# wearable-motion-capture/arm-pose-estimation

Measured on AMD Instinct MI355X. Metric: IMU windows/sec, higher is better.
Workload: dtype f32; 1 GPU; BASELINE configs[2]: watch_phone_pocket_lstm path, 1024 windows/GPU x 64 frames x 22 features (I=22,H=256,L=2,O=14), z-score+LSTM+head+denorm+FK, inputs resident in HBM; windows_per_gpu=1024, frames=64, features=22

## Files before the change

arm-pose-estimation_amd/csrc/lstm_cluster32.hip:

```cpp
#include <type_traits>

#include "ape_internal.h"
#include "async_look.h"
#include "../../include/ape_hip.h"

namespace {

typedef float f32x16 __attribute__((ext_vector_type(16)));
typedef unsigned u32x4 __attribute__((__vector_size__(4 * sizeof(unsigned))));
constexpr unsigned SPIN_LIMIT = 1u << 22;

#ifdef APE_CLUSTER_STAMPS
#define C32_TL(i) do { if (p.dbg_wg != nullptr && tid == 0 && cluster == 0 && member == 0 && (i) < 200) p.dbg_wg[256 + (i)] = __builtin_readcyclecounter(); } while (0)
#else
#define C32_TL(i) do {} while (0)
#endif

__device__ __forceinline__ float sigm(float v) { return __builtin_amdgcn_rcpf(1.0f + __builtin_amdgcn_exp2f(-1.4426950408889634f * v)); }
__device__ __forceinline__ float tanh_(float v) { return 2.0f * __builtin_amdgcn_rcpf(1.0f + __builtin_amdgcn_exp2f(-2.885390081777927f * v)) - 1.0f; }

template <bool AG>
__device__ __forceinline__ void mfma32(f32x16& acc, float w, float a) {
    if constexpr (AG) asm volatile("v_mfma_f32_32x32x2_f32 %0, %1, %2, %0" : "+v"(acc) : "a"(w), "v"(a));
    else asm volatile("v_mfma_f32_32x32x2_f32 %0, %1, %2, %0" : "+v"(acc) : "v"(w), "v"(a));
}
__device__ __forceinline__ void mfma_drain(f32x16& acc) { asm volatile("s_nop 15\n\ts_nop 7" : "+v"(acc)); }
template <bool AG>
__device__ __forceinline__ void mfma16(f32x16& acc, const u32x4& w, const u32x4& b) {
    if constexpr (AG) asm volatile("v_mfma_f32_32x32x16_f16 %0, %1, %2, %0" : "+v"(acc) : "a"(w), "v"(b));
    else asm volatile("v_mfma_f32_32x32x16_f16 %0, %1, %2, %0" : "+v"(acc) : "v"(w), "v"(b));
}

template <int NB, bool AG, int NW, typename Mid>
__device__ __forceinline__ void span32(f32x16& acc, const float* __restrict__ src, int stride, const float (&w)[NW], int w0, Mid&& mid) {
    f32x4 a0 = *reinterpret_cast<const f32x4*>(src);
    f32x4 a1 = (NB > 1) ? *reinterpret_cast<const f32x4*>(src + stride) : a0;
    f32x4 a2 = a1;
#pragma unroll
    for (int kb = 0; kb < NB; ++kb) {
        if (kb + 2 < NB) a2 = *reinterpret_cast<const f32x4*>(src + stride * (kb + 2));
#pragma unroll
        for (int j = 0; j < 4; ++j) mfma32<AG>(acc, w[w0 + 4 * kb + j], a0[j]);
        mid(kb);
        a0 = a1;
        a1 = a2;
    }
}

template <int NS, bool AG, int NG, typename Mid>
__device__ __forceinline__ void span16(f32x16& acc, const float* __restrict__ src, const u32x4 (&w)[NG], int g0, Mid&& mid) {
    constexpr int SL = 2 * 2 * 32 * 4;
    u32x4 h0 = *reinterpret_cast<const u32x4*>(src), l0 = *reinterpret_cast<const u32x4*>(src + 128);
    u32x4 h1 = (NS > 1) ? *reinterpret_cast<const u32x4*>(src + SL) : h0, l1 = (NS > 1) ? *reinterpret_cast<const u32x4*>(src + SL + 128) : l0;
    u32x4 h2 = h1, l2 = l1;
#pragma unroll
    for (int s = 0; s < NS; ++s) {
        if (s + 2 < NS) {
            h2 = *reinterpret_cast<const u32x4*>(src + SL * (s + 2));
            l2 = *reinterpret_cast<const u32x4*>(src + SL * (s + 2) + 128);
        }
        mfma16<AG>(acc, w[g0 + 2 * s], h0);
        mfma16<AG>(acc, w[g0 + 2 * s], l0);
        mid(2 * s);
        mfma16<AG>(acc, w[g0 + 2 * s + 1], h0);
        mid(2 * s + 1);
        h0 = h1; l0 = l1;
        h1 = h2; l1 = l2;
    }
}

template <bool HOT>
__device__ __forceinline__ void dma_1k(unsigned lds_addr, unsigned voff, u32x4 rsrc, unsigned soff, int piece_bytes) {
    if constexpr (HOT) {
        unsigned tmp;
        asm volatile("s_add_i32 m0, %1, %5\n\ts_add_i32 %0, %4, %5\n\tbuffer_load_dwordx4 %2, %3, %0 offen sc1 lds"
                     : "=&s"(tmp) : "s"(lds_addr), "v"(voff), "s"(rsrc), "s"(soff), "i"(piece_bytes) : "memory");
    } else {
        asm volatile("s_mov_b32 m0, %0\n\ts_nop 3\n\tbuffer_load_dwordx4 %1, %2, %3 offen sc1 lds"
                     :: "s"(lds_addr + (unsigned)piece_bytes), "v"(voff), "s"(rsrc), "s"(soff + (unsigned)piece_bytes) : "memory");
    }
}


#ifndef C32_QF
#define C32_QF 3
#endif
#ifndef C32_QPD
#define C32_QPD 0
#endif
template <int H, int L, int KX, bool ENDS, int BXU>
__global__ __launch_bounds__(256, 1) void ape_lstm_cluster32(const ClusterParams p) {
    constexpr int UPW = 8;
    constexpr int GH = H / (4 * UPW);
    constexpr int MR = 32;
    constexpr int SX = KX + 4;
    constexpr int BX = KX / 8, BH = H / 8;
    constexpr int NW0 = 4 * (BX + BH);
    constexpr int NW1 = 4 * (2 * BH);
    constexpr int NFL = 4 * GH;
    constexpr int HL = GH * 4 * MR * 8;
    constexpr int NDMA = HL * 4 / 1024 / 4;
    static_assert(H == 256 && L == 2 && KX == 32 && GH == 8 && NDMA == 8, "built for the 2 x 256 models");
    static_assert(BXU == BX || (BXU == BX - 1 && !ENDS), "the short-window instantiation keeps the four-block input span");

    const int tid = threadIdx.x;
    const int lane = tid & 63;
    const int wave = __builtin_amdgcn_readfirstlane(tid >> 6);
    const int n = lane & 31, hh = lane >> 5;
    const int T = p.T, I = p.I, O = p.O;
    const bool normalize = (p.flags & APE_FLAG_NORMALIZE_INPUT) != 0;
    const bool bcast_x = (p.flags & APE_FLAG_BROADCAST_X) != 0;

    extern __shared__ __attribute__((aligned(16))) float smem[];
    float* hb0 = smem;
    float* hb1 = hb0 + 2 * HL;
    float* xin = hb1 + HL;
    f32x4* bias_s = reinterpret_cast<f32x4*>(xin + MR * SX);
    unsigned* look_s = reinterpret_cast<unsigned*>(bias_s + 4 * L * 4 * 64);
    int* ctl = reinterpret_cast<int*>(look_s + 4 * 64);

    unsigned* const class_ticket = p.xcc_slots + 64;
    unsigned* const xcc_words = p.xcc_slots + 64 + 8 * 16;
    const int cls = blockIdx.x & 7;
    unsigned my_xcc;
    asm volatile("s_getreg_b32 %0, hwreg(HW_REG_XCC_ID)" : "=s"(my_xcc));
    my_xcc &= 0xFu;
    if (tid == 0) {
        ctl[0] = 0;
        ctl[1] = -1;
        if (__hip_atomic_load(p.status, __ATOMIC_RELAXED, __HIP_MEMORY_SCOPE_AGENT) == 0u) {
            const unsigned tk = __hip_atomic_fetch_add(class_ticket + cls * 16, 1u, __ATOMIC_RELAXED, __HIP_MEMORY_SCOPE_AGENT);
            if (tk < gridDim.x / 8) ctl[1] = (int)tk;
            else __hip_atomic_store(p.status, 2u, __ATOMIC_RELAXED, __HIP_MEMORY_SCOPE_AGENT);
        }
    }
    __syncthreads();
    if (ctl[1] < 0) return;
    const int ticket = __builtin_amdgcn_readfirstlane(ctl[1]);
    const int cluster = (ticket / GH) * 8 + cls, member = ticket % GH;
    const int row0 = cluster * MR;
    C32_TL(0);
    if (tid == 0)
        __hip_atomic_store(xcc_words + cluster * GH + member, 0x10u | my_xcc, __ATOMIC_RELAXED, __HIP_MEMORY_SCOPE_AGENT);

    constexpr int NE = (MR * KX) / 256;
    const int xk = tid % KX, xrow = tid / KX;
    const int rows_here = bcast_x ? MR : max(0, min(MR, p.B - row0));
    const unsigned long long x_addr = reinterpret_cast<unsigned long long>(p.x + (bcast_x ? (size_t)0 : (size_t)row0 * T * I));
    const unsigned x_lo = __builtin_amdgcn_readfirstlane((unsigned)x_addr), x_hi = __builtin_amdgcn_readfirstlane((unsigned)(x_addr >> 32));
    const int x_bytes = __builtin_amdgcn_readfirstlane((int)((size_t)(bcast_x ? 1 : rows_here) * T * I * sizeof(float)));
    const __amdgpu_buffer_rsrc_t x_rsrc = __builtin_amdgcn_make_buffer_rsrc(
        reinterpret_cast<float*>(((unsigned long long)x_hi << 32) | x_lo), 0, x_bytes, 0x00020000);
    const unsigned x_rowbytes = bcast_x ? 0u : (unsigned)(T * I * sizeof(float));
    const unsigned x_off0 = (xk < I) ? (unsigned)xrow * x_rowbytes + (unsigned)(xk * sizeof(float)) : 0x80000000u;
    const unsigned x_estride = (unsigned)(256 / KX) * x_rowbytes;
    float xr[NE];
    auto fetch_x = [&](int t) {
        const int slot = (t + p.x_ring >= T) ? t + p.x_ring - T : t + p.x_ring;
#pragma unroll
        for (int e = 0; e < NE; ++e) {
            const unsigned off = (xrow + e * (256 / KX) < rows_here) ? x_off0 + (unsigned)e * x_estride : 0x80000000u;
            xr[e] = __builtin_bit_cast(float, __builtin_amdgcn_raw_buffer_load_b32(x_rsrc, off, (unsigned)(slot * I * sizeof(float)), 0));
        }
    };
    double x_mean = (normalize && xk < I) ? p.xx_m[xk] : 0.0;
    double x_std = (normalize && xk < I) ? p.xx_s[xk] : 1.0;
    double x_rstd = (normalize && xk < I) ? p.xx_r[xk] : 1.0;
    asm volatile("" : "+v"(x_mean), "+v"(x_std), "+v"(x_rstd));
    auto stage_x = [&]() {
#pragma unroll
        for (int e = 0; e < NE; ++e) {
            const double d = (double)xr[e] - x_mean;
            const double q0 = d * x_rstd;
            const double rr = fma(-q0, x_std, d);
            const double q1 = fma(rr, x_rstd, q0);
            xin[(xrow + e * (256 / KX)) * SX + xk] = (float)((rr == rr) ? q1 : q0);
        }
    };
    fetch_x(0);

    float w0[4 * BXU];
    u32x4 w0h[NW0 / 4 - BX];
    u32x4 w1[NW1 / 4];
    const f32x4* const s0 = reinterpret_cast<const f32x4*>(p.wcl[0]) + ((size_t)(member * 4 + wave) * (NW0 / 4)) * 64 + lane;
    const u32x4* const s1 = reinterpret_cast<const u32x4*>(p.wcl[1]) + ((size_t)(member * 4 + wave) * (NW1 / 4)) * 64 + lane;
#pragma unroll
    for (int i = 0; i < BXU; ++i) {
        const f32x4 v = s0[i * 64];
        w0[4 * i] = v[0]; w0[4 * i + 1] = v[1]; w0[4 * i + 2] = v[2]; w0[4 * i + 3] = v[3];
    }
    auto load_weights = [&]() {
#pragma unroll
        for (int i = BX; i < NW0 / 4; ++i) w0h[i - BX] = reinterpret_cast<const u32x4*>(s0)[i * 64];
#pragma unroll
        for (int i = 0; i < NW1 / 4; ++i) w1[i] = s1[i * 64];
    };
#pragma unroll
    for (int l = 0; l < L; ++l)
#pragma unroll
        for (int gate = 0; gate < 4; ++gate) {
            f32x4 bv;
#pragma unroll
            for (int j = 0; j < 4; ++j) bv[j] = p.bias[l][gate * H + member * 32 + wave * 8 + 4 * hh + j] * p.gate_scale[l];
            bias_s[((wave * L + l) * 4 + gate) * 64 + lane] = bv;
        }
    float cst[L][4];
#pragma unroll
    for (int l = 0; l < L; ++l)
#pragma unroll
        for (int j = 0; j < 4; ++j) cst[l][j] = 0.0f;

    const __amdgpu_buffer_rsrc_t hx_rsrc = __builtin_amdgcn_make_buffer_rsrc(p.hx, 0, (int)p.hx_bytes, 0x00020000);
    const unsigned long long hx_addr = reinterpret_cast<unsigned long long>(p.hx);
    u32x4 hx_desc;
    hx_desc[0] = __builtin_amdgcn_readfirstlane((unsigned)hx_addr);
    hx_desc[1] = __builtin_amdgcn_readfirstlane((unsigned)(hx_addr >> 32) & 0xFFFFu);
    hx_desc[2] = __builtin_amdgcn_readfirstlane((unsigned)p.hx_bytes);
    hx_desc[3] = 0x00020000u;
    unsigned* const flags_of = p.xflags + (size_t)cluster * L * NFL;
    const ape_desc_t fl_desc = ape_make_desc(p.xflags, (unsigned)((gridDim.x / GH) * L * NFL * sizeof(unsigned)));
    const unsigned fl_off = (unsigned)(cluster * L * NFL * sizeof(unsigned));
    const unsigned look_voff = (unsigned)((lane & (NFL - 1)) * sizeof(unsigned));
    const unsigned look_lds = (unsigned)reinterpret_cast<unsigned long long>(look_s) + (unsigned)(wave * 256);
    const unsigned* const look_mine = look_s + wave * 64 + lane;
    constexpr unsigned SET_BYTES = HL * sizeof(float);
    auto hx_base = [&](int l, int par) -> unsigned { return (unsigned)((((size_t)cluster * L + l) * 2 + par) * SET_BYTES); };
    const unsigned hb0_lds = (unsigned)reinterpret_cast<unsigned long long>(hb0);
    const unsigned hb1_lds = (unsigned)reinterpret_cast<unsigned long long>(hb1);

    stage_x();
    if (T > 1) fetch_x(1);

    if (wave == 0) {
        unsigned spins = 0, v = 0u;
        while (true) {
            v = 0x10u | my_xcc;
            if (lane < GH) v = __hip_atomic_load(xcc_words + cluster * GH + lane, __ATOMIC_RELAXED, __HIP_MEMORY_SCOPE_AGENT);
            if (__all((int)(v != 0u))) break;
            if (++spins > SPIN_LIMIT || __hip_atomic_load(p.status, __ATOMIC_RELAXED, __HIP_MEMORY_SCOPE_AGENT) != 0u) {
                if (lane == 0) {
                    ctl[0] = 1;
                    __hip_atomic_store(p.status, 1u, __ATOMIC_RELAXED, __HIP_MEMORY_SCOPE_AGENT);
                }
                break;
            }
            __builtin_amdgcn_s_sleep(2);
        }
        const int same = __all((int)((v & 0xFu) == my_xcc));
        if (lane == 0) ctl[3] = same;
    }
    __syncthreads();
    if (ctl[0] != 0) return;
    C32_TL(1);
    const bool in_l2 = APE_HANDOVER_IN_L2(p.flags, ctl[3] != 0);

    auto wait_flags = [&](int l, unsigned want) {
        unsigned spins = 0;
        while (true) {
            unsigned v = want;
            if (lane < NFL) v = __hip_atomic_load(flags_of + l * NFL + lane, __ATOMIC_RELAXED, __HIP_MEMORY_SCOPE_AGENT);
            if (__all((int)(v >= want))) return;
            if (++spins > SPIN_LIMIT || __hip_atomic_load(p.status, __ATOMIC_RELAXED, __HIP_MEMORY_SCOPE_AGENT) != 0u) {
                if (lane == 0) {
                    ctl[0] = 1;
                    __hip_atomic_store(p.status, 1u, __ATOMIC_RELAXED, __HIP_MEMORY_SCOPE_AGENT);
                }
                return;
            }
            __builtin_amdgcn_s_sleep(1);
        }
    };
    const unsigned dma_voff = (unsigned)(lane * 16);
    auto opaque = [](unsigned v) -> unsigned { asm volatile("" : "+s"(v)); return v; };
    const unsigned wave_kib = (unsigned)(wave * 1024);
    auto issue_piece = [&](auto hot_tag, int l, int step, int k) {
        constexpr bool HOT = decltype(hot_tag)::value;
        const unsigned wk = HOT ? wave_kib : opaque(wave_kib);
        const unsigned src = hx_base(l, step & 1) + wk;
        const unsigned dst = (l == 0 ? hb0_lds + (unsigned)((step & 1) * SET_BYTES) : hb1_lds) + wk;
        dma_1k<HOT>(dst, dma_voff, hx_desc, src, k * 4096);
    };
    constexpr std::true_type HOT{};
    constexpr std::false_type COLD{};
    int pend_idx = -1;
    unsigned pend_epoch = 0u;
    auto raise_pending = [&]() {
        if (pend_idx < 0) return;
        if (lane == 0) __hip_atomic_store(flags_of + pend_idx, pend_epoch, __ATOMIC_RELAXED, __HIP_MEMORY_SCOPE_AGENT);
        pend_idx = -1;
    };
    auto bar = [&]() { asm volatile("s_waitcnt lgkmcnt(0)\n\ts_barrier" ::: "memory"); };

    auto cell_update = [&](const f32x16& acc, int l, float (&c_)[4], float (&hn)[4]) {
        const float ks = -1.4426950408889634f * p.gate_descale[l], kt = -2.885390081777927f * p.gate_descale[l];
#pragma unroll
        for (int j = 0; j < 4; j += 2) {
            typedef float f32x2 __attribute__((ext_vector_type(2)));
            auto exp2_2 = [](f32x2 v) { return f32x2{__builtin_amdgcn_exp2f(v[0]), __builtin_amdgcn_exp2f(v[1])}; };
            auto rcp_2 = [](f32x2 v) { return f32x2{__builtin_amdgcn_rcpf(v[0]), __builtin_amdgcn_rcpf(v[1])}; };
            const f32x2 ai = {acc[j], acc[j + 1]}, af = {acc[4 + j], acc[5 + j]}, ag = {acc[8 + j], acc[9 + j]}, ao = {acc[12 + j], acc[13 + j]};
            const f32x2 iv = rcp_2(1.0f + exp2_2(ks * ai));
            const f32x2 fv = rcp_2(1.0f + exp2_2(ks * af));
            const f32x2 gv = 2.0f * rcp_2(1.0f + exp2_2(kt * ag)) - 1.0f;
            const f32x2 ov = rcp_2(1.0f + exp2_2(ks * ao));
            const f32x2 c = fv * f32x2{c_[j], c_[j + 1]} + iv * gv;
            c_[j] = c[0]; c_[j + 1] = c[1];
            const f32x2 h = ov * (2.0f * rcp_2(1.0f + exp2_2(-2.885390081777927f * c)) - 1.0f);
            hn[j] = h[0]; hn[j + 1] = h[1];
        }
    };
    const unsigned pub_off = (unsigned)((((member * 4 + wave) * MR + n) * 8 + 4 * hh) * sizeof(float));
    const unsigned pub_off_split = (unsigned)(((member * 4 + wave) * 2 * MR + hh * MR + n) * 16);
    auto split_h = [&](const float (&h)[4]) -> u32x4 {
        unsigned hw[2], lw[2];
#pragma unroll
        for (int d = 0; d < 2; ++d) {
            const float a = h[2 * d] * (float)(1 << APE_C32_HSHIFT), b = h[2 * d + 1] * (float)(1 << APE_C32_HSHIFT);
            const _Float16 ah = (_Float16)a, bh = (_Float16)b;
            const _Float16 al = (_Float16)(a - (float)ah), bl = (_Float16)(b - (float)bh);
            hw[d] = (unsigned)__builtin_bit_cast(unsigned short, ah) | ((unsigned)__builtin_bit_cast(unsigned short, bh) << 16);
            lw[d] = (unsigned)__builtin_bit_cast(unsigned short, al) | ((unsigned)__builtin_bit_cast(unsigned short, bl) << 16);
        }
        u32x4 r;
#pragma unroll
        for (int d = 0; d < 2; ++d) {
            const auto sw = __builtin_amdgcn_permlane32_swap(hw[d], lw[d], false, false);
            r[d] = sw[0];
            r[2 + d] = sw[1];
        }
        return r;
    };

    if constexpr (!ENDS) {
        load_weights();
    } else {
        f32x16 acc;
#pragma unroll
        for (int gate = 0; gate < 4; ++gate) {
            const f32x4 bv = bias_s[((wave * L + 0) * 4 + gate) * 64 + lane];
            acc[4 * gate] = bv[0]; acc[4 * gate + 1] = bv[1]; acc[4 * gate + 2] = bv[2]; acc[4 * gate + 3] = bv[3];
        }
        span32<BXU, false, 4 * BXU>(acc, xin + n * SX + hh * 4, 8, w0, 0, [&](int) {});
        mfma_drain(acc);
        float h0[4];
        cell_update(acc, 0, cst[0], h0);
        const u32x4 hv = split_h(h0);
        if (in_l2) __builtin_amdgcn_raw_buffer_store_b128(hv, hx_rsrc, hx_base(0, 0) + pub_off_split, 0, 0);
        else __builtin_amdgcn_raw_buffer_store_b128(hv, hx_rsrc, hx_base(0, 0) + pub_off_split, 0, 16 );
        asm volatile("s_waitcnt vmcnt(0)" ::: "memory");
        if (lane == 0) __hip_atomic_store(flags_of + member * 4 + wave, 1u, __ATOMIC_RELAXED, __HIP_MEMORY_SCOPE_AGENT);
        asm volatile("" ::: "memory");
        load_weights();
        bar();
        if (1 < T) {
            stage_x();
            if (2 < T) fetch_x(2);
        }
    }
    C32_TL(2);

    const int P = T + L - 1;
    bool prefetched = false;
#ifdef APE_C32_COUNTS
    unsigned lc_block[2] = {0u, 0u}, lc_go[2] = {0u, 0u}, lc_n[2] = {0u, 0u};
    unsigned long long lc_top[2] = {0ull, 0ull}, lc_t0 = 0ull;
    const unsigned long long lc_start = __builtin_amdgcn_s_memtime();
#endif
#ifdef APE_CLUSTER_STAMPS
    unsigned long long dg_block[2] = {0, 0}, dg_go[2] = {0, 0};
    unsigned long long dgh[2][6] = {};
    unsigned long long dgc[2][5] = {};
    auto now = [&]() -> unsigned long long {
        const unsigned long long c = __builtin_readcyclecounter();
        asm volatile("s_waitcnt lgkmcnt(0)" ::: "memory");
        return c;
    };
#endif
    auto section = [&](auto steady_tag, auto layer_tag, auto mode_tag, const int ph) -> bool {
        constexpr bool ST = decltype(steady_tag)::value;
        constexpr int l = decltype(layer_tag)::value;
        constexpr int MODE = decltype(mode_tag)::value;
        static_assert(MODE == 0 || (l == L - 1 && (MODE == 3 || !ST)), "the special forms are layer 1's");
        const int t = ph - l;
        const bool active = ST || (t >= 0 && t < T);
        const bool need = ST || (t >= 1 && t <= T);
#ifdef APE_CLUSTER_STAMPS
        const unsigned long long c0 = ST ? now() : 0ull;
#endif
#ifdef APE_C32_COUNTS
        lc_t0 = __builtin_amdgcn_s_memtime();
#endif
        if (MODE == 3) {
        } else if (need) {
            if (!prefetched) {
#ifdef APE_CLUSTER_STAMPS
                dg_block[l] += 1;
#endif
#ifdef APE_C32_COUNTS
                lc_block[l] += 1u;
#endif
                asm volatile("s_waitcnt vmcnt(0)" ::: "memory");
                raise_pending();
                wait_flags(l, (unsigned)t);
#pragma unroll
                for (int k = 0; k < NDMA; ++k) issue_piece(COLD, l, t - 1, k);
                asm volatile("s_waitcnt vmcnt(0)" ::: "memory");
            } else {
                asm volatile("s_waitcnt vmcnt(1)" ::: "memory");
            }
        }
        prefetched = false;
#ifdef APE_CLUSTER_STAMPS
        const unsigned long long c1 = ST ? now() : 0ull;
#endif
        if constexpr (MODE != 3) bar();
#ifdef APE_CLUSTER_STAMPS
        const unsigned long long c2 = ST ? now() : 0ull;
#endif
#ifdef APE_C32_COUNTS
        if (ST && MODE != 3) { lc_top[l] += __builtin_amdgcn_s_memtime() - lc_t0; lc_n[l] += 1u; }
#endif
        const int abort_word = (MODE == 3) ? 0 : ctl[0];
        C32_TL(8 + 2 * (2 * ph + l));
        constexpr int ln = (l + 1 < L) ? l + 1 : 0;
        const int tn = (l + 1 < L) ? t - 1 : t + L;
        const bool pre = (l == L - 1) && (ST || (tn >= 1 && tn <= T));
        unsigned peek = (unsigned)tn;
        bool go = false;
        constexpr int NBL = (l == 0) ? BXU + BH : 2 * BH;
        constexpr int QF = C32_QF, QP = (MODE == 1) ? 16 : NBL / 2 - 2 + C32_QPD, QJ = (MODE == 1) ? 20 : NBL / 2 + 2 + C32_QPD;
        bool staged = false;
#ifdef APE_CLUSTER_STAMPS
        unsigned long long hk0 = 0, hk_free = 0;
#define HK_BEGIN() do { if (ST) hk0 = now(); } while (0)
#define HK_END(k) do { if (ST) dgh[l][k] += now() - hk0; } while (0)
#else
#define HK_BEGIN() do {} while (0)
#define HK_END(k) do {} while (0)
#endif
        auto mid = [&](int q) {
#ifdef APE_CLUSTER_STAMPS
            if (ST && q == QF + 2) hk_free = now();
            if (ST && q == QF + 10) dgh[l][5] += now() - hk_free;
#endif
            if (q == QF) {
                HK_BEGIN();
                asm volatile("s_waitcnt vmcnt(0)" ::: "memory");
                raise_pending();
                HK_END(0);
            }
            if (l == L - 1 && q == ((MODE == 3) ? BH + 1 : QF + 1) && (ST || ph + 1 < T)) {
                HK_BEGIN();
                stage_x();
                if (ST || ph + 2 < T) fetch_x(ph + 2);
                staged = true;
                HK_END(1);
            }
            if constexpr (l == L - 1) {
                if (q == QP) look_issue(look_lds, look_voff, fl_desc, fl_off + (unsigned)(ln * NFL * sizeof(unsigned)));
                if (q == QJ - 1) {
                    look_landed();
                    peek = *look_mine;
                }
                if (q == QJ) {
                    HK_BEGIN();
                    go = pre && __all((int)(peek >= (unsigned)tn)) != 0;
                    HK_END(2);
                }
                if (q >= QJ && q < QJ + NDMA && go) {
                    HK_BEGIN();
                    issue_piece(HOT, ln, tn - 1, q - QJ);
                    HK_END(3);
                }
            }
        };
        float hnew[4] = {0.0f, 0.0f, 0.0f, 0.0f};
        if (active) {
            f32x16 acc;
#pragma unroll
            for (int gate = 0; gate < 4; ++gate) {
                const f32x4 bv = bias_s[((wave * L + l) * 4 + gate) * 64 + lane];
                acc[4 * gate] = bv[0]; acc[4 * gate + 1] = bv[1]; acc[4 * gate + 2] = bv[2]; acc[4 * gate + 3] = bv[3];
            }
            const int frag = hh * 2 * MR * 4 + n * 4;
            if constexpr (l == 0) {
                span32<BXU, false, 4 * BXU>(acc, xin + n * SX + hh * 4, 8, w0, 0, [&](int q) { mid(q); });
                if (ST || t > 0) span16<BH / 2, false, NW0 / 4 - BX>(acc, hb0 + ((t - 1) & 1) * HL + frag, w0h, 0, [&](int q) { mid(BXU + q); });
            } else if constexpr (MODE == 3) {
                constexpr int QO = QF + 1, QO2 = QO + 12;
                static_assert(QO2 + 4 + NDMA <= QP && QP < BH, "the own gather's hooks sit in front of the look for the next section");
                unsigned pk = (unsigned)t;
                bool got1 = false, got2 = false;
                span16<BH / 2, true, NW1 / 4>(acc, hb0 + (t & 1) * HL + frag, w1, 0, [&](int q) {
                    mid(q);
                    if (q == QO) look_issue(look_lds, look_voff, fl_desc, fl_off + (unsigned)(l * NFL * sizeof(unsigned)));
                    if (q == QO + 3) {
                        look_landed();
                        pk = *look_mine;
                    }
                    if (q == QO + 4) got1 = __all((int)(pk >= (unsigned)t)) != 0;
                    if (q >= QO + 4 && q < QO + 4 + NDMA && got1) issue_piece(HOT, l, t - 1, q - (QO + 4));
                    if constexpr (!ST) {
                        if (q == QO2 && !got1) look_issue(look_lds, look_voff, fl_desc, fl_off + (unsigned)(l * NFL * sizeof(unsigned)));
                        if (q == QO2 + 3 && !got1) {
                            look_landed();
                            pk = *look_mine;
                        }
                        if (q == QO2 + 4 && !got1) got2 = __all((int)(pk >= (unsigned)t)) != 0;
                        if (q >= QO2 + 4 && q < QO2 + 4 + NDMA && got2) issue_piece(HOT, l, t - 1, q - (QO2 + 4));
                    }
                });
#ifdef APE_C32_COUNTS
                lc_t0 = __builtin_amdgcn_s_memtime();
#endif
                if (!got1 && !got2) {
#ifdef APE_CLUSTER_STAMPS
                    dg_block[l] += 1;
#endif
#ifdef APE_C32_COUNTS
                    lc_block[l] += 1u;
#endif
                    asm volatile("s_waitcnt vmcnt(0)" ::: "memory");
                    raise_pending();
                    wait_flags(l, (unsigned)t);
#pragma unroll
                    for (int k = 0; k < NDMA; ++k) issue_piece(COLD, l, t - 1, k);
                }
                asm volatile("s_waitcnt vmcnt(0)" ::: "memory");
                bar();
#ifdef APE_C32_COUNTS
                if (ST) { lc_top[l] += __builtin_amdgcn_s_memtime() - lc_t0; lc_n[l] += 1u; }
#endif
                if (ctl[0] != 0) return false;
                span16<BH / 2, true, NW1 / 4>(acc, hb1 + frag, w1, BH, [&](int q) { mid(BH + q); });
            } else {
                span16<BH / 2, true, NW1 / 4>(acc, hb0 + (t & 1) * HL + frag, w1, 0, [&](int q) { mid(q); });
                if (ST || t > 0) span16<BH / 2, true, NW1 / 4>(acc, hb1 + frag, w1, BH, [&](int q) { mid(BH + q); });
            }
#ifdef APE_CLUSTER_STAMPS
            const unsigned long long c3 = ST ? now() : 0ull;
            if (ST) { dgc[l][0] += c1 - c0; dgc[l][1] += c2 - c1; dgc[l][2] += c3 - c2; }
#endif
            mfma_drain(acc);
            cell_update(acc, l, cst[l], hnew);
        }
        if (abort_word != 0) return false;
        if (!ST && pend_idx >= 0) {
            asm volatile("s_waitcnt vmcnt(0)" ::: "memory");
            raise_pending();
        }
        if (go) prefetched = true;
#ifdef APE_CLUSTER_STAMPS
        if (go) dg_go[ln] += 1;
#endif
#ifdef APE_C32_COUNTS
        if (go) lc_go[ln] += 1u;
#endif
        if constexpr (l == L - 1) {
            if (!ST && !staged && ph + 1 < T) {
                stage_x();
                if (ph + 2 < T) fetch_x(ph + 2);
            }
        }
        {
            const bool head_only = (l == L - 1) && !ST && t == T - 1;
            const u32x4 hs = split_h(hnew);
            const u32x4 hv = head_only ? u32x4{__builtin_bit_cast(unsigned, hnew[0]), __builtin_bit_cast(unsigned, hnew[1]),
                                               __builtin_bit_cast(unsigned, hnew[2]), __builtin_bit_cast(unsigned, hnew[3])} : hs;
            const unsigned off = active ? hx_base(l, t & 1) + (head_only ? pub_off : pub_off_split) : 0x80000000u;
            if (in_l2) __builtin_amdgcn_raw_buffer_store_b128(hv, hx_rsrc, off, 0, 0);
            else __builtin_amdgcn_raw_buffer_store_b128(hv, hx_rsrc, off, 0, 16 );
            if (active) {
                pend_idx = l * NFL + member * 4 + wave;
                pend_epoch = (unsigned)(t + 1);
            }
        }
#ifdef APE_CLUSTER_STAMPS
        if (ST) { dgc[l][3] += now() - c2; dgc[l][4] += 1; }
#endif
        C32_TL(9 + 2 * (2 * ph + l));
        return true;
    };
    bool ok = true;
#pragma unroll 1
    for (int ph = ENDS ? 1 : 0; ph < P && ok; ++ph) {
        const bool st0 = ph >= 2 && ph <= T - 3, st1 = st0;
        using M0 = std::integral_constant<int, 0>;
        using L0 = std::integral_constant<int, 0>;
        using L1 = std::integral_constant<int, 1>;
        ok = st0 ? section(std::true_type{}, L0{}, M0{}, ph) : section(std::false_type{}, L0{}, M0{}, ph);
        if (!ok) break;
        const int t1 = ph - 1;
        bool done1 = false;
        if constexpr (ENDS) {
            if (!st1 && t1 == 0 && T > 1) {
                ok = section(std::false_type{}, L1{}, std::integral_constant<int, 1>{}, ph);
                done1 = true;
            }
        }
        using M3 = std::integral_constant<int, 3>;
        if (!done1 && t1 >= 1 && t1 < T) {
            ok = st1 ? section(std::true_type{}, L1{}, M3{}, ph) : section(std::false_type{}, L1{}, M3{}, ph);
            done1 = true;
        }
        if (!done1) ok = section(std::false_type{}, L1{}, M0{}, ph);
    }
    if (!ok) return;
    {
        asm volatile("s_waitcnt vmcnt(0)" ::: "memory");
        bar();
        if (pend_idx >= 0) {
            if (wave == 0 && lane < 4)
                __hip_atomic_store(flags_of + (pend_idx - wave) + lane, pend_epoch, __ATOMIC_RELAXED, __HIP_MEMORY_SCOPE_AGENT);
            pend_idx = -1;
        }
        if (!prefetched) {
            wait_flags(L - 1, (unsigned)T);
#pragma unroll
            for (int k = 0; k < NDMA; ++k) issue_piece(COLD, L - 1, T - 1, k);
        }
        asm volatile("s_waitcnt vmcnt(0)" ::: "memory");
        bar();
        if (ctl[0] != 0) return;
        C32_TL(4);
    }

#ifdef APE_CLUSTER_STAMPS
    if (p.dbg_wg != nullptr && tid == 0 && cluster == 0 && member == 0)
        for (int k = 0; k < 2; ++k) { p.dbg_wg[16 + k] = dg_block[k]; p.dbg_wg[18 + k] = dg_go[k]; }
    if (p.dbg_wg != nullptr && lane == 0 && cluster == 0 && member == 0)
        for (int l = 0; l < 2; ++l)
            for (int k = 0; k < 5; ++k) p.dbg_wg[32 + wave * 16 + l * 5 + k] = dgc[l][k];
    if (p.dbg_wg != nullptr && lane == 0 && cluster == 0 && member == 0)
        for (int l = 0; l < 2; ++l)
            for (int k = 0; k < 6; ++k) p.dbg_wg[128 + wave * 16 + l * 6 + k] = dgh[l][k];
#endif
#ifdef APE_C32_COUNTS
    if (p.dbg_wg != nullptr && tid == 0 && cluster < 24) {
        unsigned long long* o = p.dbg_wg + 512 + (cluster * GH + member) * 8;
        o[0] = lc_block[0]; o[1] = lc_block[1]; o[2] = lc_go[0]; o[3] = lc_go[1];
        o[4] = lc_top[0]; o[5] = lc_top[1]; o[6] = lc_n[0]; o[7] = __builtin_amdgcn_s_memtime() - lc_start;
    }
#endif
    {
        constexpr int RPM = MR / GH;
        const int part = tid & 3;
        for (int oi = tid >> 2; oi < ((RPM * O + 63) / 64) * 64; oi += 64) {
            const bool live = oi < RPM * O;
            const int rr = live ? oi / O : 0, o = live ? oi - rr * O : 0;
            const int row = member * RPM + rr, b = row0 + row;
            float s_acc = 0.0f;
            if (live) {
                const float* wv = p.w_out + (size_t)o * H;
                for (int kb = part; kb < H / 8; kb += 4) {
                    const f32x4 a0 = *reinterpret_cast<const f32x4*>(hb1 + kb * MR * 8 + row * 8);
                    const f32x4 a1 = *reinterpret_cast<const f32x4*>(hb1 + kb * MR * 8 + row * 8 + 4);
                    const f32x4 u0 = *reinterpret_cast<const f32x4*>(wv + kb * 8), u1 = *reinterpret_cast<const f32x4*>(wv + kb * 8 + 4);
#pragma unroll
                    for (int j = 0; j < 4; ++j) s_acc = fmaf(a0[j], u0[j], s_acc);
#pragma unroll
                    for (int j = 0; j < 4; ++j) s_acc = fmaf(a1[j], u1[j], s_acc);
                }
            }
            s_acc += __shfl_xor(s_acc, 1, 64);
            s_acc += __shfl_xor(s_acc, 2, 64);
            if (p.y != nullptr && live && part == 0 && b < p.B) p.y[(size_t)b * O + o] = s_acc + p.b_out[o];
        }
    }
    C32_TL(5);
    __syncthreads();
    if (tid == 0)
        ctl[2] = (__hip_atomic_fetch_add(p.done, 1u, __ATOMIC_RELAXED, __HIP_MEMORY_SCOPE_AGENT) == gridDim.x - 1) ? 1 : 0;
    __syncthreads();
    if (ctl[2] != 0) {
        const int n_flags = (int)(gridDim.x / GH) * L * NFL;
        for (int i = tid; i < n_flags; i += 256) __hip_atomic_store(p.xflags + i, 0u, __ATOMIC_RELAXED, __HIP_MEMORY_SCOPE_AGENT);
        for (int i = tid; i < (int)gridDim.x; i += 256) __hip_atomic_store(xcc_words + i, 0u, __ATOMIC_RELAXED, __HIP_MEMORY_SCOPE_AGENT);
        if (tid < 8) __hip_atomic_store(class_ticket + tid * 16, 0u, __ATOMIC_RELAXED, __HIP_MEMORY_SCOPE_AGENT);
        if (tid == 0) __hip_atomic_store(p.done, 0u, __ATOMIC_RELAXED, __HIP_MEMORY_SCOPE_AGENT);
    }
}

constexpr size_t smem_bytes32() {
    return ((size_t)3 * 8 * 4 * 32 * 8 + (size_t)32 * 36) * sizeof(float) + (size_t)4 * 2 * 4 * 64 * 16 + (size_t)4 * 64 * sizeof(unsigned) + 16;
}

}

bool ape_cluster32_supported(int H, int L, int KX) { return H == 256 && L == 2 && KX == 32; }

hipError_t ape_prepare_lstm_cluster32(int H, int L, int KX) {
    if (!ape_cluster32_supported(H, L, KX)) return hipSuccess;
    static_assert(smem_bytes32() <= APE_LDS_BYTES, "LDS layout exceeds a CU");
    hipError_t e = hipFuncSetAttribute(reinterpret_cast<const void*>(&ape_lstm_cluster32<256, 2, 32, false, 3>),
                                       hipFuncAttributeMaxDynamicSharedMemorySize, APE_LDS_BYTES);
    if (e != hipSuccess) return e;
    e = hipFuncSetAttribute(reinterpret_cast<const void*>(&ape_lstm_cluster32<256, 2, 32, false, 4>),
                            hipFuncAttributeMaxDynamicSharedMemorySize, APE_LDS_BYTES);
    if (e != hipSuccess) return e;
    return hipFuncSetAttribute(reinterpret_cast<const void*>(&ape_lstm_cluster32<256, 2, 32, true, 4>),
                               hipFuncAttributeMaxDynamicSharedMemorySize, APE_LDS_BYTES);
}

hipError_t ape_launch_lstm_cluster32(int H, int L, int KX, int clusters, const ClusterParams& p, hipStream_t stream) {
    if (!ape_cluster32_supported(H, L, KX)) return hipErrorInvalidValue;
    const int grid_clusters = (clusters + 7) / 8 * 8;
    constexpr size_t smem = smem_bytes32();
    if (p.T <= APE_C32_ENDS_MAX_T) hipLaunchKernelGGL((ape_lstm_cluster32<256, 2, 32, true, 4>), dim3(grid_clusters * 8), dim3(256), smem, stream, p);
    else if (p.I <= 24) hipLaunchKernelGGL((ape_lstm_cluster32<256, 2, 32, false, 3>), dim3(grid_clusters * 8), dim3(256), smem, stream, p);
    else hipLaunchKernelGGL((ape_lstm_cluster32<256, 2, 32, false, 4>), dim3(grid_clusters * 8), dim3(256), smem, stream, p);
    return hipGetLastError();
}
```

Before: 3.088 million windows/s.

## Double-buffer LSTM input and precompute next-step input projection while waiting on flags

```diff
diff --git a/arm-pose-estimation_amd/csrc/lstm_cluster32.hip b/arm-pose-estimation_amd/csrc/lstm_cluster32.hip
--- a/arm-pose-estimation_amd/csrc/lstm_cluster32.hip
+++ b/arm-pose-estimation_amd/csrc/lstm_cluster32.hip
@@ -87,6 +87,21 @@
 #endif
 #ifndef C32_QPD
 #define C32_QPD 0
+#endif
+#ifndef C32_XS
+#define C32_XS 1
+#endif
+#ifndef C32_QFP
+#define C32_QFP 12
+#endif
+#ifndef C32_QPX
+#define C32_QPX 33
+#endif
+#ifndef C32_QJX
+#define C32_QJX 54
+#endif
+#if defined(APE_C32_COUNTS) && defined(APE_C32_WAITS)
+#error "APE_C32_COUNTS and APE_C32_WAITS write the same words of dbg_wg: one build, one of them"
 #endif
 template <int H, int L, int KX, bool ENDS, int BXU>
 __global__ __launch_bounds__(256, 1) void ape_lstm_cluster32(const ClusterParams p) {
@@ -115,8 +130,9 @@
     float* hb0 = smem;
     float* hb1 = hb0 + 2 * HL;
     float* xin = hb1 + HL;
-    f32x4* bias_s = reinterpret_cast<f32x4*>(xin + MR * SX);
-    unsigned* look_s = reinterpret_cast<unsigned*>(bias_s + 4 * L * 4 * 64);
+    f32x4* bias_s = reinterpret_cast<f32x4*>(xin + 2 * MR * SX);
+    f32x4* park_s = bias_s + 4 * L * 4 * 64;
+    unsigned* look_s = reinterpret_cast<unsigned*>(park_s + 4 * 4 * 64);
     int* ctl = reinterpret_cast<int*>(look_s + 4 * 64);
 
     unsigned* const class_ticket = p.xcc_slots + 64;
@@ -167,16 +183,18 @@
     double x_std = (normalize && xk < I) ? p.xx_s[xk] : 1.0;
     double x_rstd = (normalize && xk < I) ? p.xx_r[xk] : 1.0;
     asm volatile("" : "+v"(x_mean), "+v"(x_std), "+v"(x_rstd));
-    auto stage_x = [&]() {
+    auto stage_x = [&](int t) {
+        float* const dst = xin + (ENDS ? 0 : (t & 1) * (MR * SX));
 #pragma unroll
         for (int e = 0; e < NE; ++e) {
             const double d = (double)xr[e] - x_mean;
             const double q0 = d * x_rstd;
             const double rr = fma(-q0, x_std, d);
             const double q1 = fma(rr, x_rstd, q0);
-            xin[(xrow + e * (256 / KX)) * SX + xk] = (float)((rr == rr) ? q1 : q0);
-        }
-    };
+            dst[(xrow + e * (256 / KX)) * SX + xk] = (float)((rr == rr) ? q1 : q0);
+        }
+    };
+    constexpr int XA = ENDS ? 0 : 1;
     fetch_x(0);
 
     float w0[4 * BXU];
@@ -228,7 +246,7 @@
     const unsigned hb0_lds = (unsigned)reinterpret_cast<unsigned long long>(hb0);
     const unsigned hb1_lds = (unsigned)reinterpret_cast<unsigned long long>(hb1);
 
-    stage_x();
+    stage_x(0);
     if (T > 1) fetch_x(1);
 
     if (wave == 0) {
@@ -332,6 +350,10 @@
     };
 
     if constexpr (!ENDS) {
+        if (1 < T) {
+            stage_x(1);
+            if (2 < T) fetch_x(2);
+        }
         load_weights();
     } else {
         f32x16 acc;
@@ -353,7 +375,7 @@
         load_weights();
         bar();
         if (1 < T) {
-            stage_x();
+            stage_x(1);
             if (2 < T) fetch_x(2);
         }
     }
@@ -361,10 +383,21 @@
 
     const int P = T + L - 1;
     bool prefetched = false;
+    bool parked = false;
 #ifdef APE_C32_COUNTS
     unsigned lc_block[2] = {0u, 0u}, lc_go[2] = {0u, 0u}, lc_n[2] = {0u, 0u};
     unsigned long long lc_top[2] = {0ull, 0ull}, lc_t0 = 0ull;
     const unsigned long long lc_start = __builtin_amdgcn_s_memtime();
+#endif
+#ifdef APE_C32_WAITS
+    unsigned long long lw[4] = {0ull, 0ull, 0ull, 0ull}, lw_t0 = 0ull;
+    unsigned lw_n[3] = {0u, 0u, 0u};
+    const unsigned long long lw_start = __builtin_amdgcn_s_memtime();
+#define C32_WAIT_T0() do { if (ST) lw_t0 = __builtin_amdgcn_s_memtime(); } while (0)
+#define C32_WAIT_T1(k) do { if (ST) lw[k] += __builtin_amdgcn_s_memtime() - lw_t0; } while (0)
+#else
+#define C32_WAIT_T0() do {} while (0)
+#define C32_WAIT_T1(k) do {} while (0)
 #endif
 #ifdef APE_CLUSTER_STAMPS
     unsigned long long dg_block[2] = {0, 0}, dg_go[2] = {0, 0};
@@ -390,6 +423,7 @@
 #ifdef APE_C32_COUNTS
         lc_t0 = __builtin_amdgcn_s_memtime();
 #endif
+        if constexpr (MODE != 3) C32_WAIT_T0();
         if (MODE == 3) {
         } else if (need) {
             if (!prefetched) {
@@ -419,6 +453,9 @@
 #endif
 #ifdef APE_C32_COUNTS
         if (ST && MODE != 3) { lc_top[l] += __builtin_amdgcn_s_memtime() - lc_t0; lc_n[l] += 1u; }
+#endif
+#ifdef APE_C32_WAITS
+        if constexpr (MODE != 3) { C32_WAIT_T1(3); if (ST) lw_n[1] += 1u; }
 #endif
         const int abort_word = (MODE == 3) ? 0 : ctl[0];
         C32_TL(8 + 2 * (2 * ph + l));
@@ -428,7 +465,11 @@
         unsigned peek = (unsigned)tn;
         bool go = false;
         constexpr int NBL = (l == 0) ? BXU + BH : 2 * BH;
-        constexpr int QF = C32_QF, QP = (MODE == 1) ? 16 : NBL / 2 - 2 + C32_QPD, QJ = (MODE == 1) ? 20 : NBL / 2 + 2 + C32_QPD;
+        constexpr bool LW = ST && !ENDS && MODE == 3;
+        constexpr bool XS = LW && C32_XS != 0;
+        constexpr int QF = (!ENDS && l == 0 && C32_XS != 0) ? (ST ? BXU + C32_QFP : (C32_QF > BXU ? C32_QF : BXU)) : C32_QF;
+        constexpr int QP = (MODE == 1) ? 16 : LW ? C32_QPX : NBL / 2 - 2 + C32_QPD, QJ = (MODE == 1) ? 20 : LW ? C32_QJX : NBL / 2 + 2 + C32_QPD;
+        static_assert(!LW || (QP >= 0 && QP < QJ - 1 && QJ + NDMA <= 2 * BH), "the look, its judge and the eight pieces fit the section");
         bool staged = false;
 #ifdef APE_CLUSTER_STAMPS
         unsigned long long hk0 = 0, hk_free = 0;
@@ -443,23 +484,25 @@
             if (ST && q == QF + 2) hk_free = now();
             if (ST && q == QF + 10) dgh[l][5] += now() - hk_free;
 #endif
-            if (q == QF) {
+            if (!XS && q == QF) {
                 HK_BEGIN();
                 asm volatile("s_waitcnt vmcnt(0)" ::: "memory");
                 raise_pending();
                 HK_END(0);
             }
-            if (l == L - 1 && q == ((MODE == 3) ? BH + 1 : QF + 1) && (ST || ph + 1 < T)) {
+            if (l == L - 1 && q == ((MODE == 3) ? BH + 1 : QF + 1) && (ST || ph + 1 + XA < T)) {
                 HK_BEGIN();
-                stage_x();
-                if (ST || ph + 2 < T) fetch_x(ph + 2);
+                stage_x(ph + 1 + XA);
+                if (ST || ph + 2 + XA < T) fetch_x(ph + 2 + XA);
                 staged = true;
                 HK_END(1);
             }
             if constexpr (l == L - 1) {
                 if (q == QP) look_issue(look_lds, look_voff, fl_desc, fl_off + (unsigned)(ln * NFL * sizeof(unsigned)));
                 if (q == QJ - 1) {
+                    C32_WAIT_T0();
                     look_landed();
+                    C32_WAIT_T1(1);
                     peek = *look_mine;
                 }
                 if (q == QJ) {
@@ -476,26 +519,61 @@
         };
         float hnew[4] = {0.0f, 0.0f, 0.0f, 0.0f};
         if (active) {
+            if constexpr (XS) {
+                look_issue(look_lds, look_voff, fl_desc, fl_off + (unsigned)(l * NFL * sizeof(unsigned)));
+                f32x16 ax;
+#pragma unroll
+                for (int gate = 0; gate < 4; ++gate) {
+                    const f32x4 bv = bias_s[((wave * L + 0) * 4 + gate) * 64 + lane];
+                    ax[4 * gate] = bv[0]; ax[4 * gate + 1] = bv[1]; ax[4 * gate + 2] = bv[2]; ax[4 * gate + 3] = bv[3];
+                }
+                span32<BXU, false, 4 * BXU>(ax, xin + ((ph + 1) & 1) * (MR * SX) + n * SX + hh * 4, 8, w0, 0, [&](int) {});
+                mfma_drain(ax);
+#pragma unroll
+                for (int gate = 0; gate < 4; ++gate)
+                    park_s[(wave * 4 + gate) * 64 + lane] = f32x4{ax[4 * gate], ax[4 * gate + 1], ax[4 * gate + 2], ax[4 * gate + 3]};
+                parked = true;
+            }
+            bool from_park = false;
+            if constexpr (l == 0 && !ENDS) {
+                from_park = parked;
+                parked = false;
+            }
+            const f32x4* const start_s = from_park ? park_s + wave * 4 * 64 + lane : bias_s + (wave * L + l) * 4 * 64 + lane;
             f32x16 acc;
 #pragma unroll
             for (int gate = 0; gate < 4; ++gate) {
-                const f32x4 bv = bias_s[((wave * L + l) * 4 + gate) * 64 + lane];
+                const f32x4 bv = start_s[gate * 64];
                 acc[4 * gate] = bv[0]; acc[4 * gate + 1] = bv[1]; acc[4 * gate + 2] = bv[2]; acc[4 * gate + 3] = bv[3];
             }
             const int frag = hh * 2 * MR * 4 + n * 4;
             if constexpr (l == 0) {
-                span32<BXU, false, 4 * BXU>(acc, xin + n * SX + hh * 4, 8, w0, 0, [&](int q) { mid(q); });
+                if (!from_park) span32<BXU, false, 4 * BXU>(acc, xin + (ENDS ? 0 : (t & 1) * (MR * SX)) + n * SX + hh * 4, 8, w0, 0, [&](int q) { mid(q); });
                 if (ST || t > 0) span16<BH / 2, false, NW0 / 4 - BX>(acc, hb0 + ((t - 1) & 1) * HL + frag, w0h, 0, [&](int q) { mid(BXU + q); });
             } else if constexpr (MODE == 3) {
                 constexpr int QO = QF + 1, QO2 = QO + 12;
-                static_assert(QO2 + 4 + NDMA <= QP && QP < BH, "the own gather's hooks sit in front of the look for the next section");
+                static_assert(XS || (QO2 + 4 + NDMA <= QP && (LW || QP < BH)), "the own gather's hooks sit in front of the look for the next section");
                 unsigned pk = (unsigned)t;
                 bool got1 = false, got2 = false;
+                if constexpr (XS) {
+                    C32_WAIT_T0();
+                    look_landed();
+                    C32_WAIT_T1(0);
+                    raise_pending();
+                    pk = *look_mine;
+                    got1 = __all((int)(pk >= (unsigned)t)) != 0;
+                    span16<BH / 2, true, NW1 / 4>(acc, hb0 + (t & 1) * HL + frag, w1, 0, [&](int q) {
+                        mid(q);
+                        if (q < NDMA && got1) issue_piece(HOT, l, t - 1, q);
+                    });
+                } else
                 span16<BH / 2, true, NW1 / 4>(acc, hb0 + (t & 1) * HL + frag, w1, 0, [&](int q) {
                     mid(q);
                     if (q == QO) look_issue(look_lds, look_voff, fl_desc, fl_off + (unsigned)(l * NFL * sizeof(unsigned)));
                     if (q == QO + 3) {
+                        C32_WAIT_T0();
                         look_landed();
+                        C32_WAIT_T1(0);
                         pk = *look_mine;
                     }
                     if (q == QO + 4) got1 = __all((int)(pk >= (unsigned)t)) != 0;
@@ -513,7 +591,11 @@
 #ifdef APE_C32_COUNTS
                 lc_t0 = __builtin_amdgcn_s_memtime();
 #endif
+                C32_WAIT_T0();
                 if (!got1 && !got2) {
+#ifdef APE_C32_WAITS
+                    if (ST) lw_n[2] += 1u;
+#endif
 #ifdef APE_CLUSTER_STAMPS
                     dg_block[l] += 1;
 #endif
@@ -531,6 +613,10 @@
 #ifdef APE_C32_COUNTS
                 if (ST) { lc_top[l] += __builtin_amdgcn_s_memtime() - lc_t0; lc_n[l] += 1u; }
 #endif
+#ifdef APE_C32_WAITS
+                C32_WAIT_T1(2);
+                if (ST) lw_n[0] += 1u;
+#endif
                 if (ctl[0] != 0) return false;
                 span16<BH / 2, true, NW1 / 4>(acc, hb1 + frag, w1, BH, [&](int q) { mid(BH + q); });
             } else {
@@ -557,9 +643,9 @@
         if (go) lc_go[ln] += 1u;
 #endif
         if constexpr (l == L - 1) {
-            if (!ST && !staged && ph + 1 < T) {
-                stage_x();
-                if (ph + 2 < T) fetch_x(ph + 2);
+            if (!ST && !staged && ph + 1 + XA < T) {
+                stage_x(ph + 1 + XA);
+                if (ph + 2 + XA < T) fetch_x(ph + 2 + XA);
             }
         }
         {
@@ -642,6 +728,13 @@
         o[4] = lc_top[0]; o[5] = lc_top[1]; o[6] = lc_n[0]; o[7] = __builtin_amdgcn_s_memtime() - lc_start;
     }
 #endif
+#ifdef APE_C32_WAITS
+    if (p.dbg_wg != nullptr && tid == 0 && cluster < 24) {
+        unsigned long long* o = p.dbg_wg + 512 + (cluster * GH + member) * 8;
+        o[0] = lw[0]; o[1] = lw[1]; o[2] = lw[2]; o[3] = lw[3];
+        o[4] = lw_n[0]; o[5] = lw_n[1]; o[6] = lw_n[2]; o[7] = __builtin_amdgcn_s_memtime() - lw_start;
+    }
+#endif
     {
         constexpr int RPM = MR / GH;
         const int part = tid & 3;
@@ -682,7 +775,7 @@
 }
 
 constexpr size_t smem_bytes32() {
-    return ((size_t)3 * 8 * 4 * 32 * 8 + (size_t)32 * 36) * sizeof(float) + (size_t)4 * 2 * 4 * 64 * 16 + (size_t)4 * 64 * sizeof(unsigned) + 16;
+    return ((size_t)3 * 8 * 4 * 32 * 8 + (size_t)2 * 32 * 36) * sizeof(float) + (size_t)4 * (2 + 1) * 4 * 64 * 16 + (size_t)4 * 64 * sizeof(unsigned) + 16;
 }
 
 }
```

Result: faster. 3.159 million windows/s (median of 6 runs) (+2.3%).
